# baudm/parseq

Hardware: AMD Instinct MI355X
Metric: images/sec (32x128 crops) PARSeq-S AR+refine (higher is better)
Workload: dtype bf16x3

## Files before the change

include/parseq_hip.h:

```cpp
#ifndef PARSEQ_HIP_H_
#define PARSEQ_HIP_H_

#include <stddef.h>
#include <stdint.h>

#ifdef __cplusplus
extern "C" {
#endif

#define PARSEQ_ABI_VERSION 15

#define PARSEQ_DEC_DEPTH_MAX 4

typedef struct parseq_model parseq_model;
typedef struct parseq_plan parseq_plan;

typedef struct parseq_config {
    int32_t img_h, img_w;
    int32_t patch_h, patch_w;
    int32_t embed_dim;
    int32_t enc_depth, enc_heads, enc_mlp_ratio;
    int32_t dec_depth, dec_heads, dec_mlp_ratio;
    int32_t num_tokens;
    int32_t max_label_length;
// ... 335 lines not shown
int parseq_op_mlp(float* x, const float* gamma, const float* beta, const void* W1, const float* b1, const void* W2,
                  const float* b2, int M, void* stream);
int parseq_op_attn_fused(float* x, const float* gamma, const float* beta, const void* Wqkv, const float* bqkv, const void* Wproj,
                         const float* bproj, int M, int variant, void* stream);
int parseq_op_enc_blocks(float* x, const void* const* block_ptrs, int depth, int M, void* table_ws, void* stream);
int parseq_op_enc_head_tail(float* x, const void* images, int images_dtype, const void* wpe, const float* posb, const float* norm_w,
                            const float* norm_b, const void* wkv, const float* bkv, void* kmem, void* vmem, int M, void* stream);
int parseq_op_enc_blocks_x3(float* x, const float* master, const void* pack, int64_t master_elems, const uint32_t* offsets, int depth,
                            int M, void* table_ws, float* scratch, const uint32_t* tail_offsets, float* kmem, float* vmem, void* stream);
int parseq_op_enc_blocks_x3w(float* x, const float* master, const void* pack, int64_t master_elems, const uint32_t* offsets, int depth,
                             int M, void* table_ws, float* scratch, const uint32_t* tail_offsets, float* kmem, float* vmem, void* stream);
int parseq_op_mlp_variant(float* x, const float* gamma, const float* beta, const void* W1, const float* b1, const void* W2,
                          const float* b2, int M, int variant, void* stream);
int parseq_op_encoder_attention(const void* q, const void* k, const void* vt, void* out, int dtype, int bh, int heads,
                                void* stream);
int parseq_op_train_attention(const float* qkv, float* o, float* lse, const float* d_o, float* dqkv, float* dsum, int batch, int tokens,
                              int heads, int backward, int* route, void* stream);

int parseq_op_rotate(const parseq_rotated_image_desc* image, uint8_t* out, void* stream);

int parseq_op_augment(const parseq_augment_desc* desc, uint8_t* out, void* workspace, size_t workspace_bytes, void* stream);

enum parseq_gemm_kernel {
    PARSEQ_GEMM_NONE = -1,
    PARSEQ_GEMM_VALU = 0,
    PARSEQ_GEMM_MFMA_F32 = 1,
    PARSEQ_GEMM_BF16_KK = 2, PARSEQ_GEMM_BF16_KN = 3, PARSEQ_GEMM_BF16_NK = 4, PARSEQ_GEMM_BF16_NN = 5,
    PARSEQ_GEMM_B16_KK = 6, PARSEQ_GEMM_B16_KN = 7, PARSEQ_GEMM_B16_NK = 8, PARSEQ_GEMM_B16_NN = 9,
    PARSEQ_GEMM_A16_NN = 10,
    PARSEQ_GEMM_BOTH16_K = 11,
// ... 42 lines not shown
```

parseq_amd/_native.py:

```python
from __future__ import annotations

import ctypes as C
import os
from typing import Optional

from . import build as _build

PARSEQ_F32, PARSEQ_BF16, PARSEQ_U8, PARSEQ_BF16X3 = 0, 1, 2, 3
ARCH_PARSEQ, ARCH_VITSTR = 0, 1
FLAG_DECODE_AR, FLAG_TESTING, FLAG_LATENCY = 1, 2, 4
ABI_VERSION = 15


class ParseqConfig(C.Structure):
    _fields_ = [(n, C.c_int32) for n in (
        'img_h', 'img_w', 'patch_h', 'patch_w', 'embed_dim', 'enc_depth', 'enc_heads', 'enc_mlp_ratio',
        'dec_depth', 'dec_heads', 'dec_mlp_ratio', 'num_tokens', 'max_label_length', 'bos_id', 'eos_id', 'pad_id')]
    _fields_ += [('enc_ln_eps', C.c_float), ('dec_ln_eps', C.c_float), ('arch', C.c_int32)]


class ImageDesc(C.Structure):
    _fields_ = [('data', C.c_void_p), ('height', C.c_int32), ('width', C.c_int32), ('row_stride', C.c_int64)]


# ... 202 lines not shown
                                            C.c_float, C.c_void_p]),
    'parseq_op_ln_linear_gelu': (C.c_int, [C.c_void_p, C.c_void_p, C.c_void_p, C.c_void_p, C.c_void_p, C.c_void_p, C.c_int, C.c_int,
                                           C.c_int, C.c_void_p]),
    'parseq_op_mlp': (C.c_int, [C.c_void_p, C.c_void_p, C.c_void_p, C.c_void_p, C.c_void_p, C.c_void_p, C.c_void_p, C.c_int, C.c_void_p]),
    'parseq_op_mlp_variant': (C.c_int, [C.c_void_p, C.c_void_p, C.c_void_p, C.c_void_p, C.c_void_p, C.c_void_p, C.c_void_p, C.c_int, C.c_int, C.c_void_p]),
    'parseq_op_attn_fused': (C.c_int, [C.c_void_p, C.c_void_p, C.c_void_p, C.c_void_p, C.c_void_p, C.c_void_p, C.c_void_p, C.c_int, C.c_int, C.c_void_p]),
    'parseq_op_enc_blocks': (C.c_int, [C.c_void_p, C.POINTER(C.c_void_p), C.c_int, C.c_int, C.c_void_p, C.c_void_p]),
    'parseq_op_enc_head_tail': (C.c_int, [C.c_void_p, C.c_void_p, C.c_int, C.c_void_p, C.c_void_p, C.c_void_p, C.c_void_p, C.c_void_p, C.c_void_p,
                                         C.c_void_p, C.c_void_p, C.c_int, C.c_void_p]),
    'parseq_op_enc_blocks_x3': (C.c_int, [C.c_void_p, C.c_void_p, C.c_void_p, C.c_int64, C.POINTER(C.c_uint32), C.c_int, C.c_int, C.c_void_p,
                                         C.c_void_p, C.POINTER(C.c_uint32), C.c_void_p, C.c_void_p, C.c_void_p]),
    'parseq_op_enc_blocks_x3w': (C.c_int, [C.c_void_p, C.c_void_p, C.c_void_p, C.c_int64, C.POINTER(C.c_uint32), C.c_int, C.c_int, C.c_void_p,
                                          C.c_void_p, C.POINTER(C.c_uint32), C.c_void_p, C.c_void_p, C.c_void_p]),
    'parseq_op_encoder_attention': (C.c_int, [C.c_void_p, C.c_void_p, C.c_void_p, C.c_void_p, C.c_int, C.c_int, C.c_int,
                                              C.c_void_p]),
    'parseq_op_train_attention': (C.c_int, [C.c_void_p, C.c_void_p, C.c_void_p, C.c_void_p, C.c_void_p, C.c_void_p, C.c_int, C.c_int, C.c_int,
                                            C.c_int, C.POINTER(C.c_int), C.c_void_p]),
    'parseq_op_train_gemm': (C.c_int, [C.POINTER(TrainGemmDesc), C.POINTER(GemmRoute), C.c_void_p]),
    'parseq_op_train_linear': (C.c_int, [C.c_void_p, C.c_void_p, C.c_void_p, C.c_void_p, C.c_int, C.c_void_p, C.c_void_p, C.c_void_p, C.c_void_p, C.c_void_p,
                                         C.c_void_p, C.c_void_p, C.c_int, C.c_int, C.c_int, C.c_int, C.c_int, C.c_void_p, C.c_size_t, C.c_void_p]),
    'parseq_op_train_layernorm': (C.c_int, [C.c_void_p, C.c_void_p, C.c_void_p, C.c_void_p, C.c_int, C.c_void_p, C.c_void_p, C.c_void_p, C.c_void_p, C.c_void_p,
                                            C.c_void_p, C.c_int, C.c_int, C.c_float, C.c_int, C.c_void_p, C.c_size_t, C.c_void_p]),
}


def lib_path() -> str:
    return os.environ.get('PARSEQ_HIP_LIB', _build.LIB_PATH)


def lib() -> C.CDLL:
# ... 93 lines not shown
```

parseq_amd/csrc/decoder_attn.h:

```cpp
#pragma once
#include "common.h"

namespace pq {

constexpr int DEC_MAXL = 32;
constexpr int DEC_HD = 32;

template <typename T>
__global__ __launch_bounds__(256)
void score_table_kernel(const float* __restrict__ qself, const T* __restrict__ kvtab, float* __restrict__ stab,
                        int npos, int ntok, int E) {
    const int H = E / DEC_HD;
    const size_t total = (size_t)npos * npos * ntok * H;
    const size_t idx = (size_t)blockIdx.x * blockDim.x + threadIdx.x;
    if (idx >= total) return;
    const int h = (int)(idx % H);
    size_t r = idx / H;
    const int tok = (int)(r % ntok); r /= ntok;
    const int j = (int)(r % npos);
    const int i = (int)(r / npos);
    const float* q = qself + (size_t)i * E + h * DEC_HD;
    const T* k = kvtab + ((size_t)j * ntok + tok) * (2 * E) + h * DEC_HD;
    float s = 0.f;
#pragma unroll
// ... 246 lines not shown
__device__ __forceinline__ float f24_even(unsigned hw, unsigned lw, int i) {
    return __uint_as_float(__builtin_amdgcn_perm(hw, lw, 0x0504000cu | ((unsigned)(i & 3) << 8)));
}
__device__ __forceinline__ float f24_odd(unsigned hw, unsigned lw, int i) {
    return __uint_as_float(__builtin_amdgcn_perm(hw, lw, 0x0706000cu | ((unsigned)(i & 3) << 8)));
}
__device__ __forceinline__ void f24_unpack8(const u32x4& hi, const uint2& lo, float (&v)[8]) {
#pragma unroll
    for (int i = 0; i < 8; i += 2) {
        const unsigned lw = i < 4 ? lo.x : lo.y;
        v[i] = f24_even(hi[i >> 1], lw, i);
        v[i + 1] = f24_odd(hi[i >> 1], lw, i + 1);
    }
}

template <int E, bool QSPLIT = false>
__global__ __launch_bounds__(E)
void dec_cross_attn_ar24_kernel(const float* __restrict__ qc, const QAsm qa, const unsigned char* __restrict__ kmem, const unsigned char* __restrict__ vmem,
                                size_t plane_elems, float scale, float* __restrict__ out) {
    constexpr int H = E / DEC_HD, NK = 128, LPR = 4, KPL = 16, NL = 8;
    const int lane = threadIdx.x & 63, wid = threadIdx.x >> 6, nw = E / 64, b = blockIdx.x;
    const int kl = lane / LPR, dl = lane % LPR;
    auto over_keys_sum = [](float v) {
        v = dpp_add<0x124>(v);
        v = dpp_add<0x128>(v);
        v += __shfl_xor(v, 16, 64);
        v += __shfl_xor(v, 32, 64);
        return v;
    };
    auto over_keys_max = [](float v) {
        v = dpp_max<0x124>(v);
        v = dpp_max<0x128>(v);
        v = fmaxf(v, __shfl_xor(v, 16, 64));
        v = fmaxf(v, __shfl_xor(v, 32, 64));
        return v;
    };
    __shared__ __attribute__((aligned(16))) float qs[E];
    QOne<QSPLIT> q1;
    q_issue<QSPLIT>(qa, qc, b, E, (int)threadIdx.x, q1);
    bool first = true;
    for (int h = wid; h < H; h += nw) {
        const size_t at = (((size_t)b * H + h) * NK + kl) * DEC_HD + dl * 8;
        const unsigned char* kh = kmem + at * 2; const unsigned char* kq = kmem + plane_elems * 2 + at;
        const unsigned char* vh = vmem + at * 2; const unsigned char* vq = vmem + plane_elems * 2 + at;
        u32x4 khi[NL], vhi[NL];
        uint2 klo[NL], vlo[NL];
#pragma unroll
        for (int c = 0; c < NL; ++c) khi[c] = __builtin_nontemporal_load(reinterpret_cast<const u32x4*>(kh + (size_t)c * KPL * DEC_HD * 2));
#pragma unroll
        for (int c = 0; c < NL; ++c) { const unsigned long long t = __builtin_nontemporal_load(reinterpret_cast<const unsigned long long*>(kq + (size_t)c * KPL * DEC_HD)); klo[c] = make_uint2((unsigned)t, (unsigned)(t >> 32)); }
#pragma unroll
        for (int c = 0; c < NL; ++c) vhi[c] = __builtin_nontemporal_load(reinterpret_cast<const u32x4*>(vh + (size_t)c * KPL * DEC_HD * 2));
#pragma unroll
        for (int c = 0; c < NL; ++c) { const unsigned long long t = __builtin_nontemporal_load(reinterpret_cast<const unsigned long long*>(vq + (size_t)c * KPL * DEC_HD)); vlo[c] = make_uint2((unsigned)t, (unsigned)(t >> 32)); }
        __builtin_amdgcn_sched_barrier(0);
        if (first) {
            qs[threadIdx.x] = q_finish<QSPLIT>(qa, q1, scale);
            asm volatile("s_waitcnt lgkmcnt(0)" ::: "memory");
            __builtin_amdgcn_s_barrier();
            first = false;
        }
        float qv[8];
#pragma unroll
        for (int i = 0; i < 8; i += 4) {
            const float4 v4 = *reinterpret_cast<const float4*>(qs + h * DEC_HD + dl * 8 + i);
            qv[i] = v4.x; qv[i + 1] = v4.y; qv[i + 2] = v4.z; qv[i + 3] = v4.w;
        }
        float s[NL], mx = -INFINITY;
#pragma unroll
        for (int c = 0; c < NL; ++c) {
            float kv[8];
            f24_unpack8(khi[c], klo[c], kv);
            float d = 0.f;
#pragma unroll
            for (int i = 0; i < 8; ++i) d = fmaf(qv[i], kv[i], d);
            d = dpp_add<0xB1>(d);
            d = dpp_add<0x4E>(d);
            s[c] = d;
            mx = fmaxf(mx, d);
        }
        mx = over_keys_max(mx);
        float sum = 0.f;
#pragma unroll
        for (int c = 0; c < NL; ++c) { s[c] = expf(s[c] - mx); sum += s[c]; }
        const float inv = 1.0f / over_keys_sum(sum);
        float acc[8];
#pragma unroll
        for (int i = 0; i < 8; ++i) acc[i] = 0.f;
#pragma unroll
        for (int c = 0; c < NL; ++c) {
            const float pc = s[c] * inv;
            float vv[8];
            f24_unpack8(vhi[c], vlo[c], vv);
#pragma unroll
            for (int i = 0; i < 8; ++i) acc[i] = fmaf(pc, vv[i], acc[i]);
        }
#pragma unroll
        for (int i = 0; i < 8; ++i) acc[i] = over_keys_sum(acc[i]);
        if (kl == 0) {
            float* o = out + (size_t)b * E + h * DEC_HD + dl * 8;
            *reinterpret_cast<float4*>(o) = make_float4(acc[0], acc[1], acc[2], acc[3]);
            *reinterpret_cast<float4*>(o + 4) = make_float4(acc[4], acc[5], acc[6], acc[7]);
        }
    }
}

template <typename T>
__global__ __launch_bounds__(128)
void dec_cross_attn_multi_kernel(const float* __restrict__ qc, const T* __restrict__ kmem, const T* __restrict__ vmem,
                                 int H, int Lq, float scale, T* __restrict__ out) {
    constexpr int NK = 128, QP = DEC_MAXL;
    __shared__ float sk[NK][DEC_HD + 1];
    __shared__ float sv[DEC_HD][NK + 1];
// ... 557 lines not shown
```

parseq_amd/csrc/lib_decode.hip:

```cpp
#include "lib_internal.h"
#include "beam.h"
#include "beam_refine.h"
#include "attn_map.h"
#include "lexicon_match.h"

template <typename T_, int E_> struct TE { using T = T_; static constexpr int E = E_; };
template <typename F>
static int dispatch_t(const parseq_plan* p, F&& f) { return p->precision == PARSEQ_BF16 ? f(TE<bf16_t, 0>{}) : f(TE<float, 0>{}); }
template <typename F>
static int dispatch_te(const parseq_plan* p, F&& f) {
    return dispatch_t(p, [&](auto t) {
        using T = typename decltype(t)::T;
        switch (p->m->cfg.embed_dim) {
            case 192: return f(TE<T, 192>{});
            case 384: return f(TE<T, 384>{});
            default:  return f(TE<T, 768>{});
        }
    });
}

struct LnW { const float *g, *b; };
template <typename T> struct DecLayerW {
    LnW norm_q, norm_c, norm1, norm2;
    const T *sa_in, *sa_out, *ca_in, *ca_out, *lin1, *lin2;
// ... 34 lines not shown

struct DecPass {
    int B = 0, Lk = 1, i0 = 0, Lq = 1;
    int c0 = 0;
    const unsigned char* qmask = nullptr;
    const unsigned char* cmask = nullptr;
    const unsigned char* kpm = nullptr;
    float* logits = nullptr; int Ltot = 0;
    int argmax_mode = 0;
    const float* user_query = nullptr;
    bool fused_step_allowed = false;
    void logits_of_pass(float* out, int C) { logits = out - (size_t)i0 * C; Ltot = Lq; }
};

enum DecStep { STEP_DEEP, STEP_FUSED, STEP_PER_OP };
struct DecRoute { DecStep step; bool qsplit; };
static DecRoute dec_route(const parseq_plan* p, bool latency) {
    const parseq_model* m = p->m;
    if (m->cfg.dec_depth > 1) return {STEP_DEEP, false};
    if (!(p->wstep[0] && p->fused_step && m->classes <= 128)) return {STEP_PER_OP, false};
    return {STEP_FUSED, latency && p->qsplit && m->tokens == 128 && m->cfg.max_label_length + 1 >= DS_QS + 2};
}

static float dec_scale() { return sqrtf(1.0f / (float)DEC_HD); }

enum CaKernel { CA_MFMA_N, CA_GENERIC, CA_AR24, CA_AR, CA_MULTI_MFMA, CA_MULTI_X3, CA_MULTI };
static int ca_route(bool half, int E, int NK, int Lq, bool kv24, int nsplit, CaKernel& kern) {
    if (nsplit && (nsplit != DS_QS || NK != 128 || Lq != 1)) return fail(PARSEQ_E_STATE, "cross-attention: split q-projection outside the AR step kernels");
    if (NK != 128) kern = half && (NK + 15) / 16 <= 16 ? CA_MFMA_N : CA_GENERIC;
    else if (Lq == 1) {
        if (kv24 && (half || E != 384)) return fail(PARSEQ_E_STATE, "cross-attention: 24-bit K / V rows but no kernel for this geometry");
        if (!kv24 && nsplit && E > 384) return fail(PARSEQ_E_STATE, "cross-attention: split q-projection at embed_dim %d", E);
        kern = kv24 ? CA_AR24 : CA_AR;
    } else if (half) kern = CA_MULTI_MFMA;
    else if (g_split) kern = CA_MULTI_X3;
    else if (kv24) return fail(PARSEQ_E_STATE, "cross-attention: 24-bit K / V rows outside the bf16x3 mode");
// ... 231 lines not shown
                               p->wstep[0], y.sa_out_b, w.pos_queries, y.norm1.g, y.norm1.b, p->wstep[1], y.ca_in_b, t, qsplit ? qp : tq, p->qfold, qstats);
            HIPCHK(hipGetLastError());
        }
        if (!do_start) break;
        CHK((run_cross_attention<TS, E>(p, s, 0, B, 1, ca, qa)));
        {
            ProfScope ps_(&p->prof, T_DEC_POST, s);
            hipLaunchKernelGGL((dec_step_mlp_kernel<E, X3>), dim3(grid.x * ds_split<E>()), block, (dec_step_mlp_lds<E, X3>()), s, ca, t, p->wstep[2],
                               y.ca_out_b, y.norm2.g, y.norm2.b, c.dec_ln_eps, p->wstep[3], y.lin1_b, p->wstep[4], tq, partial, M);
            HIPCHK(hipGetLastError());
        }
    }
    return 0;
}

static DecPass cloze_pass(const parseq_plan* p, int rows, int L, float* logits) {
    DecPass a; a.B = rows; a.Lk = a.Lq = L; a.qmask = a.cmask = p->cloze; a.kpm = p->kpm; a.logits = logits; a.Ltot = L;
    return a;
}

static int refine_prep(parseq_plan* p, hipStream_t s, int rows, int L, const float* logits, int from_logits) {
    const parseq_config& c = p->m->cfg;
    return launch(refine_prep_kernel, dim3((rows + 3) / 4), dim3(256), 0, s, logits, L, p->m->classes, p->tok, LDT, p->kpm, LDT, rows, c.bos_id, c.eos_id, from_logits);
}

template <typename T, int E>
static int refine_iteration(parseq_plan* p, hipStream_t s, const DecW<T>& w, int rows, int L, float* logits, int from_logits) {
    CHK(refine_prep(p, s, rows, L, logits, from_logits));
    return decoder_pass<T, E>(p, s, w, cloze_pass(p, rows, L, logits));
}

template <typename T, int E>
static int forward_impl(parseq_plan* p, int B, int flags, int refine_iters, int num_steps, float* logits, int* out_len, hipStream_t s) {
    const parseq_config& c = p->m->cfg;
    const bool ar = flags & PARSEQ_FLAG_DECODE_AR, testing = flags & PARSEQ_FLAG_TESTING;
    const DecW<T> w = dec_weights<T>(p);
    const DecRoute route = dec_route(p, flags & PARSEQ_FLAG_LATENCY);
    DecPass a; a.B = B; a.logits = logits; a.Ltot = num_steps; a.fused_step_allowed = route.step == STEP_FUSED;
    CHK(launch(ar_init_kernel, dim3((B * LDT + 255) / 256), dim3(256), 0, s, p->tok, LDT, B, c.bos_id, c.pad_id, p->eos_seen, p->counters, 2, num_steps));
    bool stepwise = ar;
    if constexpr (E <= 384) {
        if (ar && route.step == STEP_FUSED) { CHK((ar_loop_fused<E, sizeof(T) == 4>(p, s, w, B, num_steps, logits, testing, route.qsplit))); stepwise = false; }
    }
    for (int i = 0; stepwise && i < num_steps; ++i) {
        a.Lk = i + 1; a.i0 = a.c0 = i; a.Lq = 1; a.argmax_mode = i + 1 < num_steps ? (testing ? 2 : 1) : 0;
        CHK((decoder_pass<T, E>(p, s, w, a)));
    }
    if (!ar) {
        a.Lk = 1; a.Lq = num_steps;
        CHK((decoder_pass<T, E>(p, s, w, a)));
    }
    for (int it = 0; it < refine_iters; ++it) {
        CHK((refine_iteration<T, E>(p, s, w, B, num_steps, logits, (ar && it == 0) ? 0 : 1)));
    }
    int L = num_steps;
    if (ar && testing && refine_iters == 0) {
        int cnt[2];
// ... 705 lines not shown
```

parseq_amd/csrc/lib_internal.h:

```cpp
#pragma once
#include "../../include/parseq_hip.h"

#include <hip/hip_runtime.h>

#include <algorithm>
#include <cmath>
#include <cstdarg>
#include <cstdio>
#include <cstdlib>
#include <cstring>
#include <string>
#include <unordered_map>
#include <vector>

#include "common.h"
#include "decoder_attn.h"
#include "decoder_step.h"
#include "encoder_attn.h"
#include "encoder_panel.h"
#include "encoder_mlp.h"
#include "encoder_attn_fused.h"
#include "encoder_blocks.h"
#include "encoder_blocks_x3.h"
#include "encoder_blocks_x3w.h"
// ... 34 lines not shown
    explicit DevGuard(int dev) {
        if (hipGetDevice(&prev) == hipSuccess && prev != dev && hipSetDevice(dev) == hipSuccess) switched = true;
    }
    ~DevGuard() { if (switched) (void)hipSetDevice(prev); }
    DevGuard(const DevGuard&) = delete;
    DevGuard& operator=(const DevGuard&) = delete;
};

inline thread_local bool g_split = false;
struct SplitScope {
    bool prev;
    explicit SplitScope(bool on) : prev(g_split) { g_split = on; }
    ~SplitScope() { g_split = prev; }
};

enum ProfTag { T_PATCH, T_LN, T_QKV, T_ATTN, T_PROJ, T_FC1, T_FC2, T_MLP, T_ATTNF, T_BLOCKS, T_KVMEM, T_DEC_SA, T_DEC_GEMM, T_DEC_CA, T_DEC_LN, T_DEC_MISC, T_DEC_PRE, T_DEC_POST, T_COUNT };
static const char* const kProfNames[T_COUNT] = {"enc.patch_embed_gemm", "enc.layernorm", "enc.qkv_gemm", "enc.attention", "enc.proj_gemm",
                                                "enc.fc1_gelu_gemm", "enc.fc2_gemm", "enc.mlp_fused", "enc.attn_fused", "enc.blocks_fused", "dec.memory_kv_gemm", "dec.self_attention", "dec.gemm",
                                                "dec.cross_attention", "dec.layernorm", "dec.misc", "dec.step_pre", "dec.step_post"};
struct Profiler {
    bool enabled = false;
    std::vector<hipEvent_t> pool;
    std::vector<int> tags;
    size_t used = 0;
    double total_ms[T_COUNT] = {0};
    long long launches[T_COUNT] = {0};
    int begin(int tag, hipStream_t s) {
        if (!enabled) return -1;
        if ((used + 1) * 2 > pool.size()) {
            hipEvent_t a, b;
            if (hipEventCreate(&a) != hipSuccess || hipEventCreate(&b) != hipSuccess) return -1;
            pool.push_back(a); pool.push_back(b);
        }
        if (tags.size() <= used) tags.resize(used + 1);
// ... 143 lines not shown
    unsigned char* qmask_user = nullptr;
    int* counters = nullptr;
    void* kmem_l[PARSEQ_DEC_DEPTH_MAX] = {};
    void* vmem_l[PARSEQ_DEC_DEPTH_MAX] = {};
    void* kvself[PARSEQ_DEC_DEPTH_MAX] = {};
    float* xc = nullptr;
    unsigned char* cmask_user = nullptr;
    int last_batch = 0;
    bool kv24 = false;
    size_t kv_plane_elems = 0;
    bool kv24_enabled = getenv("PARSEQ_NO_KV24") == nullptr;
    int num_cus = 256;
    bool fused_step = getenv("PARSEQ_NO_FUSED_STEP") == nullptr;
    float* qfold = nullptr;
    bool qsplit = getenv("PARSEQ_NO_QSPLIT") == nullptr;
    bool fused_blocks = getenv("PARSEQ_NO_FUSED_BLOCKS") == nullptr;
    bool fused_x3 = getenv("PARSEQ_NO_FUSED_X3") == nullptr;
    int small_batch_max = [] { const char* e = getenv("PARSEQ_SMALL_BATCH"); const int v = e ? atoi(e) : 64; return v < 0 ? 0 : v; }();
    bool x3_four_waves = getenv("PARSEQ_X3_FOUR_WAVES") != nullptr;
    EncBlockParams* blocks_dev = nullptr;
    std::vector<EncBlockParams> blocks_host;
    EncTailParams enc_tail{0, 0, 0, 0, nullptr, nullptr, 0};
    bool fused_tail = getenv("PARSEQ_NO_FUSED_TAIL") == nullptr;
    float* posb = nullptr;
    unsigned wpe_off = 0;
    bool fused_head = getenv("PARSEQ_NO_FUSED_HEAD") == nullptr;
    Profiler prof;
};
constexpr int LDT = 32;

// ... 157 lines not shown
```

parseq_amd/csrc/lib_ops.hip:

```cpp
#include "lib_internal.h"
#include "eval_metrics.h"
#include "eval_beams.h"

extern "C" int parseq_postprocess(const float* logits, int batch, int L, int C, int eos_id, int32_t* ids_out, int32_t* lengths_out,
                                  float* probs_out, float* confidence_out, void* stream) {
    if (!logits || !ids_out || !lengths_out) return fail(PARSEQ_E_INVALID, "null logits / ids_out / lengths_out");
    if (batch <= 0 || L < 1 || L > 64 || C < 1) return fail(PARSEQ_E_INVALID, "bad shape: batch %d, L %d (1..64), C %d", batch, L, C);
    if (eos_id < 0 || eos_id >= C) return fail(PARSEQ_E_INVALID, "eos_id %d outside [0, %d)", eos_id, C);
    hipLaunchKernelGGL(postprocess_kernel, dim3((batch + 3) / 4), dim3(256), 0, (hipStream_t)stream, logits, batch, L, C, eos_id, ids_out,
                       lengths_out, probs_out, confidence_out);
    HIPCHK(hipGetLastError());
    return 0;
}

extern "C" int parseq_cross_entropy(const float* logits, const int32_t* targets, int rows, int C, int ignore_index, float* loss_out,
                                    int32_t* numel_out, float* workspace, void* stream) {
    if (!logits || !targets || !loss_out || !numel_out || !workspace) return fail(PARSEQ_E_INVALID, "null argument");
    if (rows <= 0 || C <= 0) return fail(PARSEQ_E_INVALID, "bad shape: rows %d, C %d", rows, C);
    hipStream_t s = (hipStream_t)stream;
    hipLaunchKernelGGL(ce_rows_kernel, dim3((rows + 3) / 4), dim3(256), 0, s, logits, targets, rows, C, ignore_index, workspace);
    HIPCHK(hipGetLastError());
    hipLaunchKernelGGL(ce_reduce_kernel, dim3(1), dim3(256), 0, s, workspace, targets, rows, ignore_index, loss_out, numel_out);
    HIPCHK(hipGetLastError());
    return 0;
// ... 317 lines not shown
    if (!x || !gamma || !beta || !W || !bias || !out || M <= 0 || N <= 0 || (N % PN_BN)) return fail(PARSEQ_E_INVALID, "bad argument (N must be a multiple of 128)");
    PanelGelu pg; pg.out = (bf16_t*)out; pg.ldo = N;
    hipStream_t s = (hipStream_t)stream;
    if (variant != 0) return fail(PARSEQ_E_INVALID, "variant %d (the ablation variants were removed)", variant);
    HIPCHK((launch_ln_panel_gemm<384, PanelGelu>(s, x, gamma, beta, 1e-6f, (const bf16_t*)W, bias, M, N, pg)));
    return 0;
}

extern "C" int parseq_op_encoder_attention(const void* q, const void* k, const void* vt, void* out, int dtype, int bh, int heads, void* stream) {
    CHK(check_arch());
    if (!q || !k || !vt || !out || bh <= 0 || heads <= 0 || bh % heads) return fail(PARSEQ_E_INVALID, "bad argument");
    if (dtype == PARSEQ_BF16) return run_enc_attention<bf16_t>((hipStream_t)stream, (const bf16_t*)q, (const bf16_t*)k, (const bf16_t*)vt, (bf16_t*)out, bh, heads);
    SplitScope ss(dtype == PARSEQ_BF16X3);
    return run_enc_attention<float>((hipStream_t)stream, (const float*)q, (const float*)k, (const float*)vt, (float*)out, bh, heads);
}
```

Baseline: 56960.

## Run the whole bf16x3 AR decode loop per row tile in one persistent kernel

Adds a persistent kernel that keeps a 16-row tile resident and runs every autoregressive step inside it: head GEMM, argmax, self-attention, cross-attention over the 24-bit K/V memory, and the MLP. Parameters stay in LDS and weights stream through a per-wave ring. This replaces per-step launches of the fused step kernels and is used when batch is at least 512 in throughput mode. The cross-attention body is factored into a shared helper, with a tiled variant and a standalone op for testing. In exchange the kernel needs a large LDS footprint and gives fewer, bigger workgroups, which could lower occupancy.

```diff
diff --git a/include/parseq_hip.h b/include/parseq_hip.h
--- a/include/parseq_hip.h
+++ b/include/parseq_hip.h
@@ -373,6 +373,8 @@
                           const float* b2, int M, int variant, void* stream);
 int parseq_op_encoder_attention(const void* q, const void* k, const void* vt, void* out, int dtype, int bh, int heads,
                                 void* stream);
+int parseq_op_cross_attention_ar24(const float* qc, const void* kmem, const void* vmem, int64_t plane_elems, int batch, int tile, float* out,
+                                   void* stream);
 int parseq_op_train_attention(const float* qkv, float* o, float* lse, const float* d_o, float* dqkv, float* dsum, int batch, int tokens,
                               int heads, int backward, int* route, void* stream);
 
diff --git a/parseq_amd/_native.py b/parseq_amd/_native.py
--- a/parseq_amd/_native.py
+++ b/parseq_amd/_native.py
@@ -240,6 +240,7 @@
                                           C.c_void_p, C.POINTER(C.c_uint32), C.c_void_p, C.c_void_p, C.c_void_p]),
     'parseq_op_encoder_attention': (C.c_int, [C.c_void_p, C.c_void_p, C.c_void_p, C.c_void_p, C.c_int, C.c_int, C.c_int,
                                               C.c_void_p]),
+    'parseq_op_cross_attention_ar24': (C.c_int, [C.c_void_p, C.c_void_p, C.c_void_p, C.c_int64, C.c_int, C.c_int, C.c_void_p, C.c_void_p]),
     'parseq_op_train_attention': (C.c_int, [C.c_void_p, C.c_void_p, C.c_void_p, C.c_void_p, C.c_void_p, C.c_void_p, C.c_int, C.c_int, C.c_int,
                                             C.c_int, C.POINTER(C.c_int), C.c_void_p]),
     'parseq_op_train_gemm': (C.c_int, [C.POINTER(TrainGemmDesc), C.POINTER(GemmRoute), C.c_void_p]),
diff --git a/parseq_amd/csrc/decoder_attn.h b/parseq_amd/csrc/decoder_attn.h
--- a/parseq_amd/csrc/decoder_attn.h
+++ b/parseq_amd/csrc/decoder_attn.h
@@ -284,12 +284,11 @@
     }
 }
 
-template <int E, bool QSPLIT = false>
-__global__ __launch_bounds__(E)
-void dec_cross_attn_ar24_kernel(const float* __restrict__ qc, const QAsm qa, const unsigned char* __restrict__ kmem, const unsigned char* __restrict__ vmem,
-                                size_t plane_elems, float scale, float* __restrict__ out) {
-    constexpr int H = E / DEC_HD, NK = 128, LPR = 4, KPL = 16, NL = 8;
-    const int lane = threadIdx.x & 63, wid = threadIdx.x >> 6, nw = E / 64, b = blockIdx.x;
+template <typename Between>
+__device__ __forceinline__ void ca24_pair(const unsigned char* __restrict__ kmem, const unsigned char* __restrict__ vmem, size_t plane_elems, size_t bh,
+                                          const float* qh, float (&acc)[8], Between&& between) {
+    constexpr int NK = 128, LPR = 4, KPL = 16, NL = 8;
+    const int lane = threadIdx.x & 63;
     const int kl = lane / LPR, dl = lane % LPR;
     auto over_keys_sum = [](float v) {
         v = dpp_add<0x124>(v);
@@ -305,68 +304,115 @@
         v = fmaxf(v, __shfl_xor(v, 32, 64));
         return v;
     };
+    const size_t at = (bh * NK + kl) * DEC_HD + dl * 8;
+    const unsigned char* kh = kmem + at * 2; const unsigned char* kq = kmem + plane_elems * 2 + at;
+    const unsigned char* vh = vmem + at * 2; const unsigned char* vq = vmem + plane_elems * 2 + at;
+    u32x4 khi[NL], vhi[NL];
+    uint2 klo[NL], vlo[NL];
+#pragma unroll
+    for (int c = 0; c < NL; ++c) khi[c] = __builtin_nontemporal_load(reinterpret_cast<const u32x4*>(kh + (size_t)c * KPL * DEC_HD * 2));
+#pragma unroll
+    for (int c = 0; c < NL; ++c) { const unsigned long long t = __builtin_nontemporal_load(reinterpret_cast<const unsigned long long*>(kq + (size_t)c * KPL * DEC_HD)); klo[c] = make_uint2((unsigned)t, (unsigned)(t >> 32)); }
+#pragma unroll
+    for (int c = 0; c < NL; ++c) vhi[c] = __builtin_nontemporal_load(reinterpret_cast<const u32x4*>(vh + (size_t)c * KPL * DEC_HD * 2));
+#pragma unroll
+    for (int c = 0; c < NL; ++c) { const unsigned long long t = __builtin_nontemporal_load(reinterpret_cast<const unsigned long long*>(vq + (size_t)c * KPL * DEC_HD)); vlo[c] = make_uint2((unsigned)t, (unsigned)(t >> 32)); }
+    __builtin_amdgcn_sched_barrier(0);
+    between();
+    float qv[8];
+#pragma unroll
+    for (int i = 0; i < 8; i += 4) {
+        const float4 v4 = *reinterpret_cast<const float4*>(qh + dl * 8 + i);
+        qv[i] = v4.x; qv[i + 1] = v4.y; qv[i + 2] = v4.z; qv[i + 3] = v4.w;
+    }
+    float s[NL], mx = -INFINITY;
+#pragma unroll
+    for (int c = 0; c < NL; ++c) {
+        float kv[8];
+        f24_unpack8(khi[c], klo[c], kv);
+        float d = 0.f;
+#pragma unroll
+        for (int i = 0; i < 8; ++i) d = fmaf(qv[i], kv[i], d);
+        d = dpp_add<0xB1>(d);
+        d = dpp_add<0x4E>(d);
+        s[c] = d;
+        mx = fmaxf(mx, d);
+    }
+    mx = over_keys_max(mx);
+    float sum = 0.f;
+#pragma unroll
+    for (int c = 0; c < NL; ++c) { s[c] = expf(s[c] - mx); sum += s[c]; }
+    const float inv = 1.0f / over_keys_sum(sum);
+#pragma unroll
+    for (int i = 0; i < 8; ++i) acc[i] = 0.f;
+#pragma unroll
+    for (int c = 0; c < NL; ++c) {
+        const float pc = s[c] * inv;
+        float vv[8];
+        f24_unpack8(vhi[c], vlo[c], vv);
+#pragma unroll
+        for (int i = 0; i < 8; ++i) acc[i] = fmaf(pc, vv[i], acc[i]);
+    }
+#pragma unroll
+    for (int i = 0; i < 8; ++i) acc[i] = over_keys_sum(acc[i]);
+}
+
+template <int E, bool QSPLIT = false>
+__global__ __launch_bounds__(E)
+void dec_cross_attn_ar24_kernel(const float* __restrict__ qc, const QAsm qa, const unsigned char* __restrict__ kmem, const unsigned char* __restrict__ vmem,
+                                size_t plane_elems, float scale, float* __restrict__ out) {
+    constexpr int H = E / DEC_HD;
+    const int lane = threadIdx.x & 63, wid = threadIdx.x >> 6, nw = E / 64, b = blockIdx.x;
+    const int kl = lane / 4, dl = lane % 4;
     __shared__ __attribute__((aligned(16))) float qs[E];
     QOne<QSPLIT> q1;
     q_issue<QSPLIT>(qa, qc, b, E, (int)threadIdx.x, q1);
     bool first = true;
     for (int h = wid; h < H; h += nw) {
-        const size_t at = (((size_t)b * H + h) * NK + kl) * DEC_HD + dl * 8;
-        const unsigned char* kh = kmem + at * 2; const unsigned char* kq = kmem + plane_elems * 2 + at;
-        const unsigned char* vh = vmem + at * 2; const unsigned char* vq = vmem + plane_elems * 2 + at;
-        u32x4 khi[NL], vhi[NL];
-        uint2 klo[NL], vlo[NL];
-#pragma unroll
-        for (int c = 0; c < NL; ++c) khi[c] = __builtin_nontemporal_load(reinterpret_cast<const u32x4*>(kh + (size_t)c * KPL * DEC_HD * 2));
-#pragma unroll
-        for (int c = 0; c < NL; ++c) { const unsigned long long t = __builtin_nontemporal_load(reinterpret_cast<const unsigned long long*>(kq + (size_t)c * KPL * DEC_HD)); klo[c] = make_uint2((unsigned)t, (unsigned)(t >> 32)); }
-#pragma unroll
-        for (int c = 0; c < NL; ++c) vhi[c] = __builtin_nontemporal_load(reinterpret_cast<const u32x4*>(vh + (size_t)c * KPL * DEC_HD * 2));
-#pragma unroll
-        for (int c = 0; c < NL; ++c) { const unsigned long long t = __builtin_nontemporal_load(reinterpret_cast<const unsigned long long*>(vq + (size_t)c * KPL * DEC_HD)); vlo[c] = make_uint2((unsigned)t, (unsigned)(t >> 32)); }
-        __builtin_amdgcn_sched_barrier(0);
-        if (first) {
-            qs[threadIdx.x] = q_finish<QSPLIT>(qa, q1, scale);
-            asm volatile("s_waitcnt lgkmcnt(0)" ::: "memory");
-            __builtin_amdgcn_s_barrier();
-            first = false;
-        }
-        float qv[8];
-#pragma unroll
-        for (int i = 0; i < 8; i += 4) {
-            const float4 v4 = *reinterpret_cast<const float4*>(qs + h * DEC_HD + dl * 8 + i);
-            qv[i] = v4.x; qv[i + 1] = v4.y; qv[i + 2] = v4.z; qv[i + 3] = v4.w;
-        }
-        float s[NL], mx = -INFINITY;
-#pragma unroll
-        for (int c = 0; c < NL; ++c) {
-            float kv[8];
-            f24_unpack8(khi[c], klo[c], kv);
-            float d = 0.f;
-#pragma unroll
-            for (int i = 0; i < 8; ++i) d = fmaf(qv[i], kv[i], d);
-            d = dpp_add<0xB1>(d);
-            d = dpp_add<0x4E>(d);
-            s[c] = d;
-            mx = fmaxf(mx, d);
-        }
-        mx = over_keys_max(mx);
-        float sum = 0.f;
-#pragma unroll
-        for (int c = 0; c < NL; ++c) { s[c] = expf(s[c] - mx); sum += s[c]; }
-        const float inv = 1.0f / over_keys_sum(sum);
         float acc[8];
-#pragma unroll
-        for (int i = 0; i < 8; ++i) acc[i] = 0.f;
-#pragma unroll
-        for (int c = 0; c < NL; ++c) {
-            const float pc = s[c] * inv;
-            float vv[8];
-            f24_unpack8(vhi[c], vlo[c], vv);
-#pragma unroll
-            for (int i = 0; i < 8; ++i) acc[i] = fmaf(pc, vv[i], acc[i]);
-        }
-#pragma unroll
-        for (int i = 0; i < 8; ++i) acc[i] = over_keys_sum(acc[i]);
+        ca24_pair(kmem, vmem, plane_elems, (size_t)b * H + h, qs + h * DEC_HD, acc, [&] {
+            if (first) {
+                qs[threadIdx.x] = q_finish<QSPLIT>(qa, q1, scale);
+                asm volatile("s_waitcnt lgkmcnt(0)" ::: "memory");
+                __builtin_amdgcn_s_barrier();
+                first = false;
+            }
+        });
+        if (kl == 0) {
+            float* o = out + (size_t)b * E + h * DEC_HD + dl * 8;
+            *reinterpret_cast<float4*>(o) = make_float4(acc[0], acc[1], acc[2], acc[3]);
+            *reinterpret_cast<float4*>(o + 4) = make_float4(acc[4], acc[5], acc[6], acc[7]);
+        }
+    }
+}
+
+constexpr int CA_TILE = 16, CA_TILE_NW = 8;
+template <int E>
+__global__ __launch_bounds__(64 * CA_TILE_NW)
+void dec_cross_attn_ar24_tile_kernel(const float* __restrict__ qc, const unsigned char* __restrict__ kmem, const unsigned char* __restrict__ vmem,
+                                     size_t plane_elems, float scale, float* __restrict__ out, int B) {
+    constexpr int H = E / DEC_HD;
+    static_assert(H > CA_TILE_NW && (CA_TILE * H) % CA_TILE_NW == 0, "every wave's first pair is of the tile's first image; equal pairs per wave");
+    const int lane = threadIdx.x & 63, wid = threadIdx.x >> 6;
+    const int kl = lane / 4, dl = lane % 4;
+    const int row0 = blockIdx.x * CA_TILE;
+    __shared__ __attribute__((aligned(16))) float qs[CA_TILE * E];
+    bool first = true;
+    for (int pr = wid; pr < CA_TILE * H; pr += CA_TILE_NW) {
+        const int img = pr / H, h = pr - img * H, b = row0 + img;
+        if (b >= B) break;
+        float acc[8];
+        ca24_pair(kmem, vmem, plane_elems, (size_t)b * H + h, qs + img * E + h * DEC_HD, acc, [&] {
+            if (first) {
+                for (int i = threadIdx.x; i < CA_TILE * (E / 4); i += 64 * CA_TILE_NW) {
+                    const int row = i / (E / 4), c = (i - row * (E / 4)) * 4;
+                    const float4 v = *reinterpret_cast<const float4*>(qc + (size_t)min(row0 + row, B - 1) * E + c);
+                    *reinterpret_cast<float4*>(qs + row * E + c) = make_float4(v.x * scale, v.y * scale, v.z * scale, v.w * scale);
+                }
+                __syncthreads();
+                first = false;
+            }
+        });
         if (kl == 0) {
             float* o = out + (size_t)b * E + h * DEC_HD + dl * 8;
             *reinterpret_cast<float4*>(o) = make_float4(acc[0], acc[1], acc[2], acc[3]);
diff --git a/parseq_amd/csrc/decoder_tile_loop.h b/parseq_amd/csrc/decoder_tile_loop.h
--- /dev/null
+++ b/parseq_amd/csrc/decoder_tile_loop.h
@@ -0,0 +1,245 @@
+#pragma once
+#include "decoder_step.h"
+
+namespace pq {
+
+struct ArTileArgs {
+    int M, num_steps, C, testing, eos_id, ldt, ntok, npos;
+    float eps, scale;
+    const float *b2, *lnf_w, *lnf_b, *bh; const bf16_t* Wh;
+    float* logits; unsigned char* eos_seen; int *eos_rows, *ar_len, *ar_last;
+    const float *stab, *kvtab; int* tok;
+    const bf16_t *Wo, *Wq; const float *bo, *pos_queries, *ln1_w, *ln1_b, *bq;
+    const unsigned char *kmem, *vmem; size_t plane_elems;
+    const bf16_t *Wco, *W1, *W2; const float *bco, *ln2_w, *ln2_b, *b1;
+};
+
+template <int E> constexpr int ds_loop_params() { return 11 * E + 128; }
+template <int E> constexpr size_t dec_ar_tile_loop_lds() {
+    return (size_t)DS_ROWS * ((E + 8) * 2 * 2 + (E + 4) * 4 + (4 * E / ds_split<E>() + 8) * 2 * 2 + 128 * 4) + (size_t)ds_loop_params<E>() * 4 + (size_t)DS_NW * DS_RING * 1024;
+}
+
+template <int E, bool X3>
+__global__ __launch_bounds__(64 * DS_NW)
+void dec_ar_tile_loop_kernel(const ArTileArgs a) {
+    static_assert(X3 && E == 384, "built for the bf16x3 arithmetic at embed_dim 384");
+    static_assert(DS_ROWS == CA_TILE && DS_NW == CA_TILE_NW, "the cross-attention's tile is the step kernels' row tile");
+    constexpr int H = E / DEC_HD, PA = E + 8, PT = E + 4, TILES = E / 16, TN = (TILES + DS_NW - 1) / DS_NW, PL = 128, RPW = DS_ROWS / DS_NW;
+    constexpr int DS_SPLIT = ds_split<E>(), F = 4 * E, FS = F / DS_SPLIT, PH = FS + 8, TN1 = FS / 16 / DS_NW;
+    static_assert(FS % (16 * DS_NW) == 0 && FS % 64 == 0, "hidden width must split evenly over the slices and waves");
+    constexpr int NPL = 2, ALO = DS_ROWS * PA, HLO = DS_ROWS * PH;
+    extern __shared__ __attribute__((aligned(16))) unsigned char smem_ds[];
+    static_assert((size_t)DS_ROWS * E * 4 <= (size_t)NPL * DS_ROWS * PH * 2 + (size_t)DS_ROWS * PL * 4, "the queries fit where they are parked");
+    const int lane = threadIdx.x & 63, wave = threadIdx.x >> 6, r16 = lane & 15, g = lane >> 4;
+    const int row0 = (int)blockIdx.x * DS_ROWS, M = a.M, C = a.C, num_steps = a.num_steps;
+    float* __restrict__ logits = a.logits;
+
+    int picked[RPW], tokv[RPW], seen[RPW];
+#pragma unroll
+    for (int rr = 0; rr < RPW; ++rr) {
+        picked[rr] = -1; seen[rr] = 0;
+        tokv[rr] = lane == 0 ? a.tok[(size_t)min(row0 + wave * RPW + rr, M - 1) * a.ldt] : 0;
+    }
+    static_assert(E <= 64 * DS_NW, "one parameter per thread and segment");
+
+#pragma unroll 1
+    for (int pos = 0; pos <= num_steps; ++pos) {
+        const bool do_start = pos < num_steps;
+        int lds0 = 0;
+        const bf16_t* Wh = a.Wh; const bf16_t* Wo = a.Wo; const bf16_t* Wq = a.Wq; const bf16_t* Wco = a.Wco; const bf16_t* W1 = a.W1; const bf16_t* W2 = a.W2;
+        const float* b1 = a.b1;
+        asm volatile("" : "+s"(lds0), "+s"(Wh), "+s"(Wo), "+s"(Wq), "+s"(Wco), "+s"(W1), "+s"(W2), "+s"(b1));
+        bf16_t* abuf = reinterpret_cast<bf16_t*>(smem_ds + lds0);
+        float* tl = reinterpret_cast<float*>(abuf + NPL * DS_ROWS * PA);
+        bf16_t* hbuf = reinterpret_cast<bf16_t*>(tl + DS_ROWS * PT);
+        float* lg = reinterpret_cast<float*>(hbuf + NPL * DS_ROWS * PH);
+        float* qs = reinterpret_cast<float*>(hbuf);
+        float* prm = lg + DS_ROWS * PL;
+        float* const s_lnf_w = prm, * const s_lnf_b = prm + E, * const s_bh = prm + 2 * E, * const s_bo = prm + 2 * E + 128, * const s_posq = prm + 3 * E + 128,
+             * const s_ln1_w = prm + 4 * E + 128, * const s_ln1_b = prm + 5 * E + 128, * const s_bq = prm + 6 * E + 128, * const s_bco = prm + 7 * E + 128,
+             * const s_ln2_w = prm + 8 * E + 128, * const s_ln2_b = prm + 9 * E + 128, * const s_b2 = prm + 10 * E + 128;
+        unsigned char* wring = reinterpret_cast<unsigned char*>(prm + ds_loop_params<E>()) + wave * DS_RING * 1024;
+        if (pos == 0) {
+            float* const prm_dst[11] = {s_lnf_w, s_lnf_b, s_bh, s_bo, s_ln1_w, s_ln1_b, s_bq, s_bco, s_ln2_w, s_ln2_b, s_b2};
+            const float* const prm_src[11] = {a.lnf_w, a.lnf_b, a.bh, a.bo, a.ln1_w, a.ln1_b, a.bq, a.bco, a.ln2_w, a.ln2_b, a.b2};
+            const int prm_n[11] = {E, E, 128, E, E, E, E, E, E, E, E}, prm_valid[11] = {E, E, C, E, E, E, E, E, E, E, E};
+            float prm_v[11];
+            ds_params_load<11>(prm_v, prm_src, prm_valid);
+            ds_params_store<11>(prm_v, prm_dst, prm_n, prm_valid);
+            ds_prefetch<E, TN, NPL>(Wo, TILES, wave, wring);
+        }
+        if (pos > 0) {
+            ds_layernorm_rows<E, X3>(tl, PT, abuf, PA, s_lnf_w, s_lnf_b, a.eps, wave, ALO);
+            __syncthreads();
+            {
+                f32x4 acc[1] = {};
+                ds_wave_gemm<E, 1, true, NPL>(abuf, PA, Wh, (C + 15) / 16, wave, wring, acc, 0, 0, ALO);
+                if (do_start) ds_prefetch<E, TN, NPL>(Wo, TILES, wave, wring);
+                const int n = wave * 16 + 4 * g;
+#pragma unroll
+                for (int r = 0; r < 4; ++r) {
+                    if (n + r < C) {
+                        const float v = acc[0][r] + s_bh[n + r];
+                        lg[r16 * PL + n + r] = v;
+                        if (row0 + r16 < M) logits[((size_t)(row0 + r16) * num_steps + (pos - 1)) * C + n + r] = v;
+                    }
+                }
+            }
+            __syncthreads();
+            if (do_start) {
+#pragma unroll
+                for (int rr = 0; rr < RPW; ++rr) {
+                    const int row = wave * RPW + rr, b = row0 + row;
+                    float best = -INFINITY; int bi = ARGMAX_NONE;
+                    for (int c = lane; c < C; c += 64) {
+                        const float v = lg[row * PL + c];
+                        if (argmax_take(v, c, best, bi)) { best = v; bi = c; }
+                    }
+                    wave_argmax(best, bi);
+                    bi = argmax_final(bi, C);
+                    picked[rr] = bi;
+                    if (lane == 0 && b < M) {
+                        a.tok[(size_t)b * a.ldt + pos] = bi;
+                        if (a.testing && bi == a.eos_id && !seen[rr]) {
+                            seen[rr] = 1; a.eos_seen[b] = 1;
+                            atomicMax(a.ar_last, pos);
+                            __threadfence();
+                            const int done = atomicAdd(a.eos_rows, 1) + 1;
+                            if (done == M) { __threadfence(); *a.ar_len = atomicMax(a.ar_last, 0); }
+                        }
+                    }
+                }
+            }
+        }
+        if (!do_start) break;
+
+        const int Lk = pos + 1;
+        if (threadIdx.x < E) s_posq[threadIdx.x] = a.pos_queries[(size_t)min(pos, a.npos - 1) * E + threadIdx.x];
+        {
+#pragma unroll
+            for (int rr = 0; rr < RPW; ++rr)
+                if (picked[rr] >= 0 && lane == pos) tokv[rr] = picked[rr];
+            ds_self_attn_rows<E, X3, RPW>(a.stab, a.kvtab, tokv, a.ntok, a.npos, Lk, pos, abuf + wave * RPW * PA, PA, ALO);
+        }
+        __syncthreads();
+        {
+            f32x4 acc[TN] = {};
+            ds_wave_gemm<E, TN, true, NPL>(abuf, PA, Wo, TILES, wave, wring, acc, 0, 0, ALO);
+            ds_prefetch<E, TN, NPL>(Wq, TILES, wave, wring);
+#pragma unroll
+            for (int t = 0; t < TN; ++t) {
+                const int tile = wave + DS_NW * t;
+                if (tile < TILES) {
+                    const int n = tile * 16 + 4 * g;
+                    const float4 bv = *reinterpret_cast<const float4*>(s_bo + n);
+                    const float4 pv = *reinterpret_cast<const float4*>(s_posq + n);
+                    f32x4 o = {acc[t][0] + bv.x + pv.x, acc[t][1] + bv.y + pv.y, acc[t][2] + bv.z + pv.z, acc[t][3] + bv.w + pv.w};
+                    *reinterpret_cast<f32x4*>(tl + r16 * PT + n) = o;
+                }
+            }
+        }
+        __syncthreads();
+        ds_layernorm_rows<E, X3>(tl, PT, abuf, PA, s_ln1_w, s_ln1_b, a.eps, wave, ALO);
+        __syncthreads();
+        {
+            f32x4 acc[TN] = {};
+            ds_wave_gemm<E, TN, true, NPL>(abuf, PA, Wq, TILES, wave, wring, acc, 0, 0, ALO);
+#pragma unroll
+            for (int t = 0; t < TN; ++t) {
+                const int tile = wave + DS_NW * t;
+                if (tile < TILES) {
+                    const int n = tile * 16 + 4 * g;
+                    const float4 bv = *reinterpret_cast<const float4*>(s_bq + n);
+                    const f32x4 o = {acc[t][0] + bv.x, acc[t][1] + bv.y, acc[t][2] + bv.z, acc[t][3] + bv.w};
+                    const f32x4 q = {o[0] * a.scale, o[1] * a.scale, o[2] * a.scale, o[3] * a.scale};
+                    *reinterpret_cast<f32x4*>(qs + r16 * E + n) = q;
+                }
+            }
+        }
+        __syncthreads();
+
+        {
+            const int kl = lane / 4, dl = lane % 4;
+#pragma unroll 1
+            for (int pr = wave; pr < DS_ROWS * H; pr += DS_NW) {
+                const int img = pr / H, h = pr - img * H, b = row0 + img;
+                if (b >= M) break;
+                float acc[8];
+                ca24_pair(a.kmem, a.vmem, a.plane_elems, (size_t)b * H + h, qs + img * E + h * DEC_HD, acc, [] {});
+                if (kl == 0) {
+                    bf16x8 hi, lo;
+#pragma unroll
+                    for (int j = 0; j < 8; ++j) { hi[j] = from_f32<bf16_t>(acc[j]); lo[j] = from_f32<bf16_t>(acc[j] - to_f32(hi[j])); }
+                    *reinterpret_cast<bf16x8*>(abuf + img * PA + h * DEC_HD + dl * 8) = hi;
+                    *reinterpret_cast<bf16x8*>(abuf + ALO + img * PA + h * DEC_HD + dl * 8) = lo;
+                }
+            }
+        }
+        ds_prefetch<E, TN, NPL>(Wco, TILES, wave, wring);
+        __syncthreads();
+        {
+            f32x4 acc[TN] = {};
+            ds_wave_gemm<E, TN, true, NPL>(abuf, PA, Wco, TILES, wave, wring, acc, 0, 0, ALO);
+            ds_prefetch<E, TN1, NPL>(W1, FS / 16, wave, wring);
+#pragma unroll
+            for (int t = 0; t < TN; ++t) {
+                const int tile = wave + DS_NW * t;
+                if (tile < TILES) {
+                    const int n = tile * 16 + 4 * g;
+                    const float4 bv = *reinterpret_cast<const float4*>(s_bco + n);
+                    f32x4* p = reinterpret_cast<f32x4*>(tl + r16 * PT + n);
+                    f32x4 o = *p;
+                    o[0] += acc[t][0] + bv.x; o[1] += acc[t][1] + bv.y; o[2] += acc[t][2] + bv.z; o[3] += acc[t][3] + bv.w;
+                    *p = o;
+                }
+            }
+        }
+        __syncthreads();
+        ds_layernorm_rows<E, X3>(tl, PT, abuf, PA, s_ln2_w, s_ln2_b, a.eps, wave, ALO);
+        __syncthreads();
+#pragma unroll 1
+        for (int sp = 0; sp < DS_SPLIT; ++sp) {
+            {
+                f32x4 acc[TN1] = {};
+                ds_wave_gemm<E, TN1, true, NPL>(abuf, PA, W1 + (size_t)sp * (FS / 16) * (E / 64) * (1024 * NPL), FS / 16, wave, wring, acc, 0, 0, ALO);
+                ds_prefetch<FS, TN, NPL>(W2, TILES, wave, wring, sp * (FS / 64), F / 64);
+#pragma unroll
+                for (int t = 0; t < TN1; ++t) {
+                    const int n = (wave + DS_NW * t) * 16 + 4 * g;
+                    const float4 bv = *reinterpret_cast<const float4*>(b1 + sp * FS + n);
+                    const float o[4] = {gelu_erf(acc[t][0] + bv.x), gelu_erf(acc[t][1] + bv.y), gelu_erf(acc[t][2] + bv.z), gelu_erf(acc[t][3] + bv.w)};
+                    float ol[4];
+#pragma unroll
+                    for (int j = 0; j < 4; ++j) ol[j] = o[j] - to_f32(from_f32<bf16_t>(o[j]));
+                    store4<bf16_t>(hbuf + r16 * PH + n, o);
+                    store4<bf16_t>(hbuf + HLO + r16 * PH + n, ol);
+                }
+            }
+            __syncthreads();
+            {
+                f32x4 acc[TN] = {};
+                ds_wave_gemm<FS, TN, true, NPL>(hbuf, PH, W2, TILES, wave, wring, acc, sp * (FS / 64), F / 64, HLO);
+                if (sp + 1 < DS_SPLIT) ds_prefetch<E, TN1, NPL>(W1 + (size_t)(sp + 1) * (FS / 16) * (E / 64) * (1024 * NPL), FS / 16, wave, wring);
+                else ds_prefetch<E, 1, NPL>(Wh, (C + 15) / 16, wave, wring);
+#pragma unroll
+                for (int t = 0; t < TN; ++t) {
+                    const int tile = wave + DS_NW * t;
+                    if (tile < TILES) {
+                        const int n = tile * 16 + 4 * g;
+                        f32x4* p = reinterpret_cast<f32x4*>(tl + r16 * PT + n);
+                        f32x4 v = *p;
+                        if (sp == 0) {
+                            const float4 bv = *reinterpret_cast<const float4*>(s_b2 + n);
+                            v[0] += bv.x; v[1] += bv.y; v[2] += bv.z; v[3] += bv.w;
+                        }
+                        v += acc[t];
+                        *p = v;
+                    }
+                }
+            }
+            __syncthreads();
+        }
+    }
+}
+
+}
diff --git a/parseq_amd/csrc/lib_decode.hip b/parseq_amd/csrc/lib_decode.hip
--- a/parseq_amd/csrc/lib_decode.hip
+++ b/parseq_amd/csrc/lib_decode.hip
@@ -1,4 +1,5 @@
 #include "lib_internal.h"
+#include "decoder_tile_loop.h"
 #include "beam.h"
 #include "beam_refine.h"
 #include "attn_map.h"
@@ -72,12 +73,14 @@
 };
 
 enum DecStep { STEP_DEEP, STEP_FUSED, STEP_PER_OP };
-struct DecRoute { DecStep step; bool qsplit; };
-static DecRoute dec_route(const parseq_plan* p, bool latency) {
+struct DecRoute { DecStep step; bool qsplit; bool tile_loop; };
+static DecRoute dec_route(const parseq_plan* p, bool latency, int batch = 0) {
     const parseq_model* m = p->m;
-    if (m->cfg.dec_depth > 1) return {STEP_DEEP, false};
-    if (!(p->wstep[0] && p->fused_step && m->classes <= 128)) return {STEP_PER_OP, false};
-    return {STEP_FUSED, latency && p->qsplit && m->tokens == 128 && m->cfg.max_label_length + 1 >= DS_QS + 2};
+    if (m->cfg.dec_depth > 1) return {STEP_DEEP, false, false};
+    if (!(p->wstep[0] && p->fused_step && m->classes <= 128)) return {STEP_PER_OP, false, false};
+    const bool tile_loop = !latency && p->tile_loop && p->precision == PARSEQ_BF16X3 && m->cfg.embed_dim == 384 && m->tokens == 128 && p->kv24 &&
+                           batch >= p->tile_loop_min;
+    return {STEP_FUSED, latency && p->qsplit && m->tokens == 128 && m->cfg.max_label_length + 1 >= DS_QS + 2, tile_loop};
 }
 
 static float dec_scale() { return sqrtf(1.0f / (float)DEC_HD); }
@@ -339,6 +342,27 @@
     return 0;
 }
 
+template <int E>
+static int ar_tile_loop(parseq_plan* p, hipStream_t s, const DecW<float>& w, int B, int num_steps, float* logits, bool testing) {
+    const parseq_config& c = p->m->cfg;
+    const DecLayerW<float>& y = w.layer[0];
+    ArTileArgs a{};
+    a.M = B; a.num_steps = num_steps; a.C = p->m->classes; a.testing = testing ? 1 : 0; a.eos_id = c.eos_id; a.ldt = LDT; a.ntok = c.num_tokens;
+    a.npos = c.max_label_length + 1; a.eps = c.dec_ln_eps; a.scale = dec_scale();
+    a.b2 = y.lin2_b; a.lnf_w = w.norm.g; a.lnf_b = w.norm.b; a.bh = w.head_b; a.Wh = p->wstep[5];
+    a.logits = logits; a.eos_seen = p->eos_seen; a.eos_rows = p->counters; a.ar_len = p->counters + 1; a.ar_last = p->counters + 2;
+    a.stab = p->stab; a.kvtab = reinterpret_cast<const float*>(p->kvtab); a.tok = p->tok;
+    a.Wo = p->wstep[0]; a.Wq = p->wstep[1]; a.bo = y.sa_out_b; a.pos_queries = w.pos_queries; a.ln1_w = y.norm1.g; a.ln1_b = y.norm1.b; a.bq = y.ca_in_b;
+    a.kmem = reinterpret_cast<const unsigned char*>(p->kmem); a.vmem = reinterpret_cast<const unsigned char*>(p->vmem); a.plane_elems = p->kv_plane_elems;
+    a.Wco = p->wstep[2]; a.W1 = p->wstep[3]; a.W2 = p->wstep[4]; a.bco = y.ca_out_b; a.ln2_w = y.norm2.g; a.ln2_b = y.norm2.b; a.b1 = y.lin1_b;
+    static LdsAttr attr_;
+    HIPCHK(attr_.ensure(reinterpret_cast<const void*>(dec_ar_tile_loop_kernel<E, true>), dec_ar_tile_loop_lds<E>()));
+    ProfScope ps_(&p->prof, T_DEC_LOOP, s);
+    hipLaunchKernelGGL((dec_ar_tile_loop_kernel<E, true>), dim3((B + DS_ROWS - 1) / DS_ROWS), dim3(64 * DS_NW), dec_ar_tile_loop_lds<E>(), s, a);
+    HIPCHK(hipGetLastError());
+    return 0;
+}
+
 static DecPass cloze_pass(const parseq_plan* p, int rows, int L, float* logits) {
     DecPass a; a.B = rows; a.Lk = a.Lq = L; a.qmask = a.cmask = p->cloze; a.kpm = p->kpm; a.logits = logits; a.Ltot = L;
     return a;
@@ -360,12 +384,19 @@
     const parseq_config& c = p->m->cfg;
     const bool ar = flags & PARSEQ_FLAG_DECODE_AR, testing = flags & PARSEQ_FLAG_TESTING;
     const DecW<T> w = dec_weights<T>(p);
-    const DecRoute route = dec_route(p, flags & PARSEQ_FLAG_LATENCY);
+    const DecRoute route = dec_route(p, flags & PARSEQ_FLAG_LATENCY, B);
     DecPass a; a.B = B; a.logits = logits; a.Ltot = num_steps; a.fused_step_allowed = route.step == STEP_FUSED;
-    CHK(launch(ar_init_kernel, dim3((B * LDT + 255) / 256), dim3(256), 0, s, p->tok, LDT, B, c.bos_id, c.pad_id, p->eos_seen, p->counters, 2, num_steps));
+    CHK(launch(ar_init_kernel, dim3((B * LDT + 255) / 256), dim3(256), 0, s, p->tok, LDT, B, c.bos_id, c.pad_id, p->eos_seen, p->counters, 3, num_steps));
     bool stepwise = ar;
     if constexpr (E <= 384) {
-        if (ar && route.step == STEP_FUSED) { CHK((ar_loop_fused<E, sizeof(T) == 4>(p, s, w, B, num_steps, logits, testing, route.qsplit))); stepwise = false; }
+        if (ar && route.step == STEP_FUSED) {
+            bool looped = false;
+            if constexpr (E == 384 && sizeof(T) == 4) {
+                if (route.tile_loop) { CHK((ar_tile_loop<E>(p, s, w, B, num_steps, logits, testing))); looped = true; }
+            }
+            if (!looped) CHK((ar_loop_fused<E, sizeof(T) == 4>(p, s, w, B, num_steps, logits, testing, route.qsplit)));
+            stepwise = false;
+        }
     }
     for (int i = 0; stepwise && i < num_steps; ++i) {
         a.Lk = i + 1; a.i0 = a.c0 = i; a.Lq = 1; a.argmax_mode = i + 1 < num_steps ? (testing ? 2 : 1) : 0;
diff --git a/parseq_amd/csrc/lib_internal.h b/parseq_amd/csrc/lib_internal.h
--- a/parseq_amd/csrc/lib_internal.h
+++ b/parseq_amd/csrc/lib_internal.h
@@ -72,10 +72,10 @@
     ~SplitScope() { g_split = prev; }
 };
 
-enum ProfTag { T_PATCH, T_LN, T_QKV, T_ATTN, T_PROJ, T_FC1, T_FC2, T_MLP, T_ATTNF, T_BLOCKS, T_KVMEM, T_DEC_SA, T_DEC_GEMM, T_DEC_CA, T_DEC_LN, T_DEC_MISC, T_DEC_PRE, T_DEC_POST, T_COUNT };
+enum ProfTag { T_PATCH, T_LN, T_QKV, T_ATTN, T_PROJ, T_FC1, T_FC2, T_MLP, T_ATTNF, T_BLOCKS, T_KVMEM, T_DEC_SA, T_DEC_GEMM, T_DEC_CA, T_DEC_LN, T_DEC_MISC, T_DEC_PRE, T_DEC_POST, T_DEC_LOOP, T_COUNT };
 static const char* const kProfNames[T_COUNT] = {"enc.patch_embed_gemm", "enc.layernorm", "enc.qkv_gemm", "enc.attention", "enc.proj_gemm",
                                                 "enc.fc1_gelu_gemm", "enc.fc2_gemm", "enc.mlp_fused", "enc.attn_fused", "enc.blocks_fused", "dec.memory_kv_gemm", "dec.self_attention", "dec.gemm",
-                                                "dec.cross_attention", "dec.layernorm", "dec.misc", "dec.step_pre", "dec.step_post"};
+                                                "dec.cross_attention", "dec.layernorm", "dec.misc", "dec.step_pre", "dec.step_post", "dec.ar_tile_loop"};
 struct Profiler {
     bool enabled = false;
     std::vector<hipEvent_t> pool;
@@ -249,6 +249,8 @@
     bool fused_step = getenv("PARSEQ_NO_FUSED_STEP") == nullptr;
     float* qfold = nullptr;
     bool qsplit = getenv("PARSEQ_NO_QSPLIT") == nullptr;
+    bool tile_loop = getenv("PARSEQ_NO_TILE_LOOP") == nullptr;
+    int tile_loop_min = [] { const char* e = getenv("PARSEQ_TILE_LOOP_MIN"); const int v = e ? atoi(e) : 512; return v < 1 ? 1 : v; }();
     bool fused_blocks = getenv("PARSEQ_NO_FUSED_BLOCKS") == nullptr;
     bool fused_x3 = getenv("PARSEQ_NO_FUSED_X3") == nullptr;
     int small_batch_max = [] { const char* e = getenv("PARSEQ_SMALL_BATCH"); const int v = e ? atoi(e) : 64; return v < 0 ? 0 : v; }();
diff --git a/parseq_amd/csrc/lib_ops.hip b/parseq_amd/csrc/lib_ops.hip
--- a/parseq_amd/csrc/lib_ops.hip
+++ b/parseq_amd/csrc/lib_ops.hip
@@ -355,3 +355,16 @@
     SplitScope ss(dtype == PARSEQ_BF16X3);
     return run_enc_attention<float>((hipStream_t)stream, (const float*)q, (const float*)k, (const float*)vt, (float*)out, bh, heads);
 }
+
+extern "C" int parseq_op_cross_attention_ar24(const float* qc, const void* kmem, const void* vmem, int64_t plane_elems, int batch, int tile, float* out, void* stream) {
+    CHK(check_arch());
+    if (!qc || !kmem || !vmem || !out) return fail(PARSEQ_E_INVALID, "cross_attention_ar24: null argument");
+    if (batch < 1) return fail(PARSEQ_E_INVALID, "cross_attention_ar24: batch %d", batch);
+    if (plane_elems < (int64_t)batch * 384 * 128) return fail(PARSEQ_E_INVALID, "cross_attention_ar24: planes of %lld elements hold fewer than %d images", (long long)plane_elems, batch);
+    if (tile != 0 && tile != 1) return fail(PARSEQ_E_INVALID, "cross_attention_ar24: tile %d (0 or 1)", tile);
+    const unsigned char* k = reinterpret_cast<const unsigned char*>(kmem); const unsigned char* v = reinterpret_cast<const unsigned char*>(vmem);
+    const float scale = sqrtf(1.0f / (float)DEC_HD);
+    if (tile) return launch(dec_cross_attn_ar24_tile_kernel<384>, dim3((batch + CA_TILE - 1) / CA_TILE), dim3(64 * CA_TILE_NW), 0, (hipStream_t)stream, qc, k, v,
+                            (size_t)plane_elems, scale, out, batch);
+    return launch(dec_cross_attn_ar24_kernel<384, false>, dim3(batch), dim3(384), 0, (hipStream_t)stream, qc, QAsm{}, k, v, (size_t)plane_elems, scale, out);
+}
```

Result: faster. 59080 (median of 6 runs) (+3.7%).
